# cg-saarland/hagrid

Measured on AMD Instinct MI355X. Metric: Mrays/s (primary traversal) + grid build ms, 1M-tri scene @1/2/4/8 MI355X, higher is better.
Workload: dtype f32

## Files before the change

hagrid_amd/csrc/ctx.h:

```cpp
#pragma once

#include <hip/hip_runtime.h>

#include <atomic>
#include <cstdio>
#include <memory>
#include <string>
#include <unordered_map>
#include <vector>

#include "hagrid_amd.h"

namespace hagrid_impl {

struct Slot {
    void* ptr = nullptr;
    size_t size = 0;
    bool in_use = false;
    int refs = 0;
};

}

namespace hagrid_impl {
// ... 60 lines not shown
enum DistanceScratch : int { kScrDistTasks = 0, kScrDistTooLarge = 1 };
enum ImageScratch : int {
    kScrImgStatus = 160,
    kScrImgLevelCounts = 164,
    kScrImgClearedWords = 24,
    kScrImgTableTotal = 224,
    kScrImgSlimStatus = 228,
};
constexpr bool scr_apart(int a, int na, int b, int nb) { return a + na <= b || b + nb <= a; }
constexpr bool scr_free(int a, int n) { return a >= 0 && a + n <= kScrRowLenBinned; }
static_assert(kScrRowLenBinned + 2 <= kScrRowLen && kScrRowLen + 4 <= kScrMaxRef && kScrMaxRef < kScrBlobFlag && kScrBlobFlag < kScratchWords, "fixed-owner words");
static_assert(kScrBuildTooLarge + 1 <= kScrBuildLevelTotals && kScrBuildShift + 8 == kScrBuildLevelTotals + 1, "build_grid: scalars and the first level's total");
static_assert(scr_apart(kScrBuildLevelTotals, 4 * kBuildMaxLevels, kScrBuildCarry, 2 * kBuildMaxLevels), "build_grid: totals and carries");
static_assert(scr_free(kScrBuildLevelTotals, 4 * kBuildMaxLevels) && scr_free(kScrBuildCarry, 2 * kBuildMaxLevels), "build_grid: level-indexed words");
static_assert(kScrMergeTotals + 6 <= kScrMergeBooks && kScrMergeBooks + 4 == kScrMergeSnapshots && kScrMergeSnapshots + 6 == kScrMergeIpTotal && scr_free(kScrMergeIpTotal, 2), "merge_grid");
static_assert(scr_free(kScrFlattenCarry, HAGRID_MAX_LEVELS + 2), "flatten_grid: a carry per group of levels");
static_assert(scr_free(kScrExpandCounts, kExpandMaxListed), "expand_grid");
static_assert(kScrDistTasks + 1 == kScrDistTooLarge && scr_free(kScrDistTasks, 2) && scr_free(kScrCompressTotal, 1), "distance_lattice (its two words are cleared together), compress_grid");
static_assert(kScrImgStatus + 3 <= kScrImgLevelCounts && kScrImgLevelCounts + kImageMaxLevels + 1 <= kScrImgStatus + kScrImgClearedWords, "setup_traversal: the general layout's words are cleared together");
static_assert(scr_apart(kScrImgStatus, kScrImgClearedWords, kScrImgTableTotal, 1) && scr_apart(kScrImgTableTotal, 1, kScrImgSlimStatus, 3) && scr_free(kScrImgSlimStatus, 3), "setup_traversal");
}

struct hagrid_ctx {
    int device = 0;
    hipStream_t stream = nullptr;
    bool keep = false;
    int num_cus = 0;

    std::vector<hagrid_impl::Slot> slots;
    std::unordered_map<void*, int> tracker;
    size_t usage = 0, max_usage = 0;

    hipEvent_t ev_begin = nullptr, ev_end = nullptr;

    int* mailbox = nullptr;
    int* dscratch = nullptr;
    unsigned long long* lb_state = nullptr;
    size_t lb_words = 0;
    unsigned lb_epoch = 0;
    int* row_scores = nullptr;
    int* bin_diff = nullptr;

    int ray_binning = 0;
    int opt_variant = 0;
    int opt_lookback = 1;
    int opt_merge_inplace = 1;
    int opt_merge_inplace_iters = 0;
    int opt_merge_inplace_div = 0;
    int opt_merge_inplace_room = 0;
    int opt_merge_narrow = 1;
    int opt_expand_voxel_map = 1;
    int opt_expand_subset_only = 1;
    int opt_expand_listed = 1;
    int opt_expand_max_listed = hagrid_impl::kExpandMaxListed;
    int opt_distance_by_triangle = 0;
    int opt_image_width = 0;
    int opt_band_rows = 0;
    int opt_super_log2 = 3;
    int opt_xcd_chunk_log2 = -2;
    int opt_narrow = 1;
    int opt_image_max_mb = 0;
    int opt_quad_head = 20;
    int opt_image_vtop = 1;
    int opt_image_uniform = 1;
    int opt_row_cache = 1;
    struct RayHints {
        const void* key_rays = nullptr; int key_n = 0;
        unsigned long long used = 0;
        struct Rows {
            const void* rowlen_rays = nullptr; int rowlen_n = 0, rowlen_age = 0;
            int rowlen_known = -1, rowlen_seen = 0;
            bool rows_from_origins = false;
            hipEvent_t rowlen_evt = nullptr; bool rowlen_pending = false;
        } rows;
        struct Order {
            int* lpt_buf = nullptr; int lpt_cap = 0;
            const void* lpt_rays = nullptr; int lpt_n = 0, lpt_blocks = 0, lpt_age = 0, lpt_period = 32;
            int lpt_rot = 0;
            bool lpt_valid = false; int lpt_epoch = 1;
            unsigned order_serial = 0; int last_report = -1;
            unsigned long long relearn_clock = 0; int cooldown = 0, cooldown_len = 64;
        } order;
        struct Trial {
            bool rot_adopted = false, head_disabled = false;
            float t_base = 0.0f, t_head = 0.0f, t_all = 0.0f; int n_base = 0, n_head = 0, n_all = 0;
            bool learned_all = false; int all_stage = 0;
            bool cmp_pending = false, cmp_done = false;
            int n_conf = 0; float t_conf = 0.0f;
        } trial;
        hipEvent_t trial_evt[2] = {nullptr, nullptr}; bool trial_pending = false; int trial_kind = 0;
        int trial_opt = -1; unsigned head_serial = 0;
        struct Share {
            hipEvent_t share_evt[12][2] = {}; int share_issued = 0, share_done = 0;
            int share_choice = -1;
            int share_ncand = 0, share_shape_nc = 0;
            int share_cands[4] = {0, 0, 0, 0}; float share_t[4] = {0.0f, 0.0f, 0.0f, 0.0f};
            int share_last = -1;
            int share_launches = 0; unsigned share_serial = 0;
            bool learned_once = false;
            bool order_loses = false;
        } share;
    };
    static constexpr int kRayHints = 4;
    RayHints hints[kRayHints];
    unsigned long long hint_clock = 0;
    int opt_mailbox = -1;
// ... 108 lines not shown
```

hagrid_amd/csrc/expand.hip:

```cpp
#include "ctx.h"
#include "wave_prims.h"

#include "hagrid/grid.h"
#include "hagrid/prims.h"

using namespace hagrid;
using namespace hagrid_impl;

namespace {

struct ExpandK { ivec3 dims; ivec3 top; int shift; vec3 gmin, cell_size, grid_inv; const int* voxel_cells; };
constexpr int kChanged = 1 << 3;
struct CellRec { ivec3 lo; int begin; ivec3 hi; int end; };

__device__ __forceinline__ CellRec load_cell(const Cell* cells, int i) {
    const int4* p = reinterpret_cast<const int4*>(cells) + 2 * size_t(i);
    const int4 a = p[0], b = p[1];
    CellRec c; c.lo = ivec3(a.x, a.y, a.z); c.begin = a.w; c.hi = ivec3(b.x, b.y, b.z); c.end = b.w;
    return c;
}
__device__ __forceinline__ int comp(const ivec3& v, int axis) { return axis == 0 ? v.x : (axis == 1 ? v.y : v.z); }


__device__ __forceinline__ int lower_bound_in(const int* __restrict__ a, int n, int x) {
    int lo = 0, hi = n;
    while (lo < hi) {
        const int mid = (lo + hi) >> 1;
        if (a[mid] < x) lo = mid + 1; else hi = mid;
    }
    return lo;
}

__device__ __forceinline__ bool contains_all(const int* __restrict__ big, int nbig, const int* __restrict__ small, int nsmall) {
    if (nsmall > nbig) return false;
    if (nsmall == 0) return true;
    if (nbig <= 4) {
        const int b0 = big[0], b1 = nbig > 1 ? big[1] : -1, b2 = nbig > 2 ? big[2] : -1, b3 = nbig > 3 ? big[3] : -1;
        const int s0 = small[0], s1 = nsmall > 1 ? small[1] : s0, s2 = nsmall > 2 ? small[2] : s0, s3 = nsmall > 3 ? small[3] : s0;
        auto in_big = [&](int x) { return (x == b0) | (x == b1) | (x == b2) | (x == b3); };
        return in_big(s0) & in_big(s1) & in_big(s2) & in_big(s3);
    }
    for (int j = 0; j < nsmall; j++) {
        const int x = small[j], at = lower_bound_in(big, nbig, x);
        if (at == nbig || big[at] != x) return false;
    }
    return true;
}

__device__ __forceinline__ Tri load_tri(const float4* __restrict__ tris, int i) {
    const float4* p = tris + 3 * size_t(i);
    const float4 a = p[0], b = p[1], c = p[2];
    return Tri(vec3(a.x, a.y, a.z), a.w, vec3(b.x, b.y, b.z), b.w, vec3(c.x, c.y, c.z), c.w);
}

__global__ void __launch_bounds__(kBlock) fill_voxel_cells(ExpandK k, const Entry* __restrict__ entries, int* __restrict__ voxel_cells, int voxels) {
    const int v = blockIdx.x * kBlock + threadIdx.x;
    if (v >= voxels) return;
    const int s = k.shift, m = (1 << s) - 1, top = v >> (3 * s), local = v & ((1 << (3 * s)) - 1);
    const int tx = top % k.top.x, ty = (top / k.top.x) % k.top.y, tz = top / (k.top.x * k.top.y);
    const ivec3 at((tx << s) + (local & m), (ty << s) + ((local >> s) & m), (tz << s) + (local >> (2 * s)));
    voxel_cells[v] = int(lookup_entry(entries, s, k.top, at));
}
__device__ __forceinline__ int cell_of_voxel(const ExpandK& k, const Entry* __restrict__ entries, const ivec3& at) {
    if (!k.voxel_cells) return int(lookup_entry(entries, k.shift, k.top, at));
    const int s = k.shift, m = (1 << s) - 1;
    const int top = (at.x >> s) + k.top.x * ((at.y >> s) + k.top.y * (at.z >> s));
    return k.voxel_cells[(top << (3 * s)) + (at.x & m) + (((at.y & m) + ((at.z & m) << s)) << s)];
}

template <int AXIS>
__device__ __forceinline__ int room_before_prim(const ExpandK& k, const Tri& prim, const CellRec& cell, const BBox& cross, int room, bool UP) {
    constexpr int A1 = (AXIS + 1) % 3, A2 = (AXIS + 2) % 3;
    const BBox pb = prim.bbox();
    const bool overlaps = get<A1>(pb.min) <= get<A1>(cross.max) && get<A1>(pb.max) >= get<A1>(cross.min) &&
                          get<A2>(pb.min) <= get<A2>(cross.max) && get<A2>(pb.max) >= get<A2>(cross.min);
    if (!overlaps) return room;
    const int layer = int(((UP ? get<AXIS>(pb.min) : get<AXIS>(pb.max)) - get<AXIS>(k.gmin)) * get<AXIS>(k.grid_inv));
    const int free_layers = UP ? layer - comp(cell.hi, AXIS) : comp(cell.lo, AXIS) - layer - 1;
    return max(min(room, free_layers), 0);
}

template <int AXIS, bool SUBSET_ONLY>
__device__ __forceinline__ int face_growth(const ExpandK& k, const Entry* __restrict__ entries, const int* __restrict__ refs, const float4* __restrict__ tris,
                                           const Cell* __restrict__ cells, const CellRec& cell, bool UP, bool& again) {
    constexpr int A1 = (AXIS + 1) % 3, A2 = (AXIS + 2) % 3;
    const int face = UP ? comp(cell.hi, AXIS) : comp(cell.lo, AXIS);
    const int extent = comp(k.dims, AXIS);
    if (UP ? face >= extent : face <= 0) return 0;
    const int layer = UP ? face : face - 1;
    const int lo1 = comp(cell.lo, A1), hi1 = comp(cell.hi, A1), lo2 = comp(cell.lo, A2), hi2 = comp(cell.hi, A2);
    const int own = cell.end - cell.begin;
    int reach = extent, room = extent;
    int u = lo1, v = lo2, row_step = comp(k.dims, A2);
    for (;;) {
        const ivec3 at = AXIS == 0 ? ivec3(layer, u, v) : (AXIS == 1 ? ivec3(v, layer, u) : ivec3(u, v, layer));
        const CellRec nb = load_cell(cells, cell_of_voxel(k, entries, at));
        reach = min(reach, UP ? comp(nb.hi, AXIS) - face : face - comp(nb.lo, AXIS));
        room = min(room, reach);
        const int theirs = nb.end - nb.begin;
        if (SUBSET_ONLY) {
            if (!contains_all(refs + cell.begin, own, refs + nb.begin, theirs)) { room = 0; break; }
        } else if (theirs > 0) {
            const BBox cross(k.gmin + k.cell_size * vec3(cell.lo), k.gmin + k.cell_size * vec3(cell.hi));
            int mine = 0;
            for (int j = 0; j < theirs && room > 0; j++) {
                const int id = refs[nb.begin + j];
                while (mine < own && refs[cell.begin + mine] < id) mine++;
                if (mine < own && refs[cell.begin + mine] == id) continue;
                room = room_before_prim<AXIS>(k, load_tri(tris, id), cell, cross, room, UP);
            }
            if (room == 0) break;
        }
        row_step = min(row_step, comp(nb.hi, A2) - v);
        u = comp(nb.hi, A1);
        if (u >= hi1) {
            u = lo1; v += row_step; row_step = comp(k.dims, A2);
            if (v >= hi2) break;
        }
    }
    again |= room == reach;
    return UP ? room : -room;
}

template <int axis, bool SUBSET_ONLY, bool PAIRED>
__device__ __forceinline__ void grow_cell(const ExpandK& k, const Entry* __restrict__ entries, const int* __restrict__ refs, const float4* __restrict__ tris,
                                          const Cell* __restrict__ cells, Cell* __restrict__ new_cells, unsigned char* __restrict__ cell_flags, int id, int flags, bool up) {
    CellRec cell = load_cell(cells, id);
    bool flag = false;
    int ov1, ov2;
    if (PAIRED) {
        bool again = false;
        const int mine = face_growth<axis, SUBSET_ONLY>(k, entries, refs, tris, cells, cell, up, again);
        const int other = __shfl_xor(mine, 1, 64);
        flag = again | (__shfl_xor(int(again), 1, 64) != 0);
        if (up) return;
        ov1 = mine; ov2 = other;
    } else {
        ov1 = face_growth<axis, SUBSET_ONLY>(k, entries, refs, tris, cells, cell, false, flag);
        ov2 = face_growth<axis, SUBSET_ONLY>(k, entries, refs, tris, cells, cell, true, flag);
    }
    if (axis == 0) { cell.lo.x += ov1; cell.hi.x += ov2; }
    if (axis == 1) { cell.lo.y += ov1; cell.hi.y += ov2; }
    if (axis == 2) { cell.lo.z += ov1; cell.hi.z += ov2; }
    cell_flags[id] = (unsigned char)((flag ? 1 << axis : 0) | (flags & ~((1 << axis) | kChanged)) | ((ov1 | ov2) ? kChanged : 0));
    int4* out = reinterpret_cast<int4*>(new_cells) + 2 * size_t(id);
    out[0] = make_int4(cell.lo.x, cell.lo.y, cell.lo.z, cell.begin);
    out[1] = make_int4(cell.hi.x, cell.hi.y, cell.hi.z, cell.end);
}

template <int axis, bool SUBSET_ONLY>
__global__ void __launch_bounds__(kBlock) overlap_step(ExpandK k, const Entry* __restrict__ entries, const int* __restrict__ refs,
                                                       const float4* __restrict__ tris, const Cell* __restrict__ cells, Cell* __restrict__ new_cells,
                                                       unsigned char* __restrict__ cell_flags, int num_cells) {
    const int id = xcd_block(blockIdx.x, gridDim.x) * kBlock + threadIdx.x;
    if (id >= num_cells) return;
    const int flags = cell_flags[id];
    if ((flags & (1 << axis)) == 0) {
        const int4* p = reinterpret_cast<const int4*>(cells) + 2 * size_t(id);
        int4* out = reinterpret_cast<int4*>(new_cells) + 2 * size_t(id);
        const int4 a = p[0], b = p[1];
        out[0] = a; out[1] = b;
        if (flags & kChanged) cell_flags[id] = (unsigned char)(flags & ~kChanged);
        return;
    }
    grow_cell<axis, SUBSET_ONLY, false>(k, entries, refs, tris, cells, new_cells, cell_flags, id, flags, false);
}

constexpr int kSelectItems = 16;
constexpr int kSelectTile = kBlock * kSelectItems;

template <int axis>
__global__ void __launch_bounds__(kBlock) expand_select(const Cell* __restrict__ cells, Cell* __restrict__ new_cells, unsigned char* __restrict__ cell_flags,
                                                        int num_cells, int* __restrict__ list, int* __restrict__ count) {
    __shared__ int tile_list[kSelectTile];
    __shared__ int tile_count, tile_base;
    if (threadIdx.x == 0) tile_count = 0;
    __syncthreads();
    const int base = blockIdx.x * kSelectTile;
    int fl[kSelectItems];
    #pragma unroll
    for (int j = 0; j < kSelectItems; j++) {
        const int id = base + j * kBlock + threadIdx.x;
        fl[j] = id < num_cells ? cell_flags[id] : 0;
    }
    #pragma unroll
    for (int j = 0; j < kSelectItems; j++) {
        const int id = base + j * kBlock + threadIdx.x;
        const int flags = fl[j];
        const bool listed = (flags & (1 << axis)) != 0;
        const unsigned long long m = __ballot(listed);
        int wbase = 0;
        if (lane_id() == 0 && m) wbase = atomicAdd(&tile_count, __popcll(m));
        wbase = __shfl(wbase, 0, 64);
        if (listed) {
            tile_list[wbase + __popcll(m & ((1ull << lane_id()) - 1ull))] = id;
        } else if (flags & kChanged) {
            const int4* p = reinterpret_cast<const int4*>(cells) + 2 * size_t(id);
            int4* out = reinterpret_cast<int4*>(new_cells) + 2 * size_t(id);
            const int4 a = p[0], b = p[1];
            out[0] = a; out[1] = b;
            cell_flags[id] = (unsigned char)(flags & ~kChanged);
        }
    }
    __syncthreads();
    if (threadIdx.x == 0) tile_base = tile_count ? atomicAdd(count, tile_count) : 0;
    __syncthreads();
    for (int i = threadIdx.x; i < tile_count; i += kBlock) list[tile_base + i] = tile_list[i];
}

template <int axis, bool SUBSET_ONLY>
__global__ void __launch_bounds__(kBlock) expand_listed(ExpandK k, const Entry* __restrict__ entries, const int* __restrict__ refs,
                                                        const float4* __restrict__ tris, const Cell* __restrict__ cells, Cell* __restrict__ new_cells,
                                                        unsigned char* __restrict__ cell_flags, const int* __restrict__ list, const int* __restrict__ count) {
    const int n = *count, active = (2 * n + kBlock - 1) / kBlock;
    if (int(blockIdx.x) >= active) return;
    const int t = xcd_block(blockIdx.x, active) * kBlock + threadIdx.x;
    const int i = t >> 1;
    if (i >= n) return;
    const int id = list[i];
    grow_cell<axis, SUBSET_ONLY, true>(k, entries, refs, tris, cells, new_cells, cell_flags, id, cell_flags[id], (t & 1) != 0);
}

template <int axis, bool SUBSET_ONLY>
void listed_step(hipStream_t st, const ExpandK& k, const Entry* entries, const int* refs, const float4* tris, const Cell* cells, Cell* other,
                 unsigned char* flags, int n, int* list, int* count) {
    expand_select<axis><<<grid_blocks(n, kSelectTile), kBlock, 0, st>>>(cells, other, flags, n, list, count);
    expand_listed<axis, SUBSET_ONLY><<<grid_blocks(2ll * n, kBlock), kBlock, 0, st>>>(k, entries, refs, tris, cells, other, flags, list, count);
}

template <bool SUBSET_ONLY>
void listed_iteration(hipStream_t st, const ExpandK& k, const Entry* entries, const int* refs, const float4* tris, Cell*& cells, Cell*& other,
                      unsigned char* flags, int n, int* list, int* counts) {
    listed_step<0, SUBSET_ONLY>(st, k, entries, refs, tris, cells, other, flags, n, list, counts + 0); std::swap(cells, other);
    listed_step<1, SUBSET_ONLY>(st, k, entries, refs, tris, cells, other, flags, n, list, counts + 1); std::swap(cells, other);
    listed_step<2, SUBSET_ONLY>(st, k, entries, refs, tris, cells, other, flags, n, list, counts + 2); std::swap(cells, other);
}
template <bool SUBSET_ONLY>
void all_cells_iteration(hagrid_ctx* ctx, const ExpandK& k, const Entry* entries, const int* refs, const float4* tris, Cell*& cells, Cell*& other,
                         unsigned char* flags, int n) {
    hipStream_t st = ctx->stream;
    const int blocks = grid_blocks(n, kBlock);
    overlap_step<0, SUBSET_ONLY><<<blocks, kBlock, 0, st>>>(k, entries, refs, tris, cells, other, flags, n); HG_DBG(ctx); std::swap(cells, other);
    overlap_step<1, SUBSET_ONLY><<<blocks, kBlock, 0, st>>>(k, entries, refs, tris, cells, other, flags, n); HG_DBG(ctx); std::swap(cells, other);
    overlap_step<2, SUBSET_ONLY><<<blocks, kBlock, 0, st>>>(k, entries, refs, tris, cells, other, flags, n); HG_DBG(ctx); std::swap(cells, other);
}

}

extern "C" int hagrid_expand_grid(hagrid_ctx* ctx, hagrid_grid* grid, const void* tris_v, int iters) {
    if (!ctx || !grid) return HAGRID_EINVAL;
    const bool subset_only = ctx->opt_expand_subset_only != 0;
    if (!subset_only && !tris_v && iters > 0) HG_FAIL(ctx, HAGRID_EINVAL, "expand_grid: the precise mode needs the triangles");
    const float4* tris = static_cast<const float4*>(tris_v);
    if (iters <= 0) return HAGRID_OK;
    if (!grid->cells || !grid->entries || !grid->ref_ids) HG_FAIL(ctx, HAGRID_EINVAL, "expand_grid: incomplete (or compressed) grid");
    trav_image_drop(ctx);
    HG_HIP(ctx, hipSetDevice(ctx->device));
    hipStream_t st = ctx->stream;
    ExpandK k;
    k.top = ivec3(grid->dims[0], grid->dims[1], grid->dims[2]);
    k.dims = k.top << grid->shift;
    k.shift = grid->shift;
    {
        const vec3 lo(grid->bbox_min[0], grid->bbox_min[1], grid->bbox_min[2]), ext = vec3(grid->bbox_max[0], grid->bbox_max[1], grid->bbox_max[2]) - lo;
        k.gmin = lo; k.cell_size = ext / vec3(k.dims); k.grid_inv = vec3(k.dims) / ext;
    }
    const int n = grid->num_cells;
    Cell* cells = static_cast<Cell*>(grid->cells);
    Cell* other = pool_alloc<Cell>(ctx, size_t(n));
    unsigned char* flags = pool_alloc<unsigned char>(ctx, size_t(n));
    if (!other || !flags) { hagrid_mem_free(ctx, other); hagrid_mem_free(ctx, flags); return HAGRID_ENOMEM; }
    (void)hipMemsetAsync(flags, 0xFF, size_t(n), st);
    const Entry* entries = static_cast<const Entry*>(grid->entries);
    const int* refs = static_cast<const int*>(grid->ref_ids);
    int* list = iters > 1 && ctx->opt_expand_listed ? pool_try_alloc<int>(ctx, size_t(n)) : nullptr;
    const long long voxels = (long long)k.dims.x * k.dims.y * k.dims.z;
    int* voxel_cells = (ctx->opt_expand_voxel_map && voxels <= (1ll << 28)) ? pool_try_alloc<int>(ctx, size_t(voxels)) : nullptr;
    k.voxel_cells = voxel_cells;
    if (voxel_cells) { ExpandK kf = k; kf.voxel_cells = nullptr; fill_voxel_cells<<<grid_blocks(voxels, kBlock), kBlock, 0, st>>>(kf, entries, voxel_cells, int(voxels)); HG_DBG(ctx); }
    int* counts = ctx->dscratch + kScrExpandCounts;
    const int max_listed = std::min(std::max(ctx->opt_expand_max_listed, 0), kExpandMaxListed);
    if (list) (void)hipMemsetAsync(counts, 0, kExpandMaxListed * sizeof(int), st);
    int listed = 0;
    for (int it = 0; it < iters; it++) {
        if (it > 0 && list && listed + 3 <= max_listed) {
            if (subset_only) listed_iteration<true>(st, k, entries, refs, tris, cells, other, flags, n, list, counts + listed);
            else             listed_iteration<false>(st, k, entries, refs, tris, cells, other, flags, n, list, counts + listed);
            listed += 3;
            continue;
        }
        if (subset_only) all_cells_iteration<true>(ctx, k, entries, refs, tris, cells, other, flags, n);
        else             all_cells_iteration<false>(ctx, k, entries, refs, tris, cells, other, flags, n);
    }
    hipError_t e = hipGetLastError();
    if (e == hipSuccess) e = hipStreamSynchronize(st);
    ctx->counts.expand_passes = 3 * iters; ctx->counts.expand_cells = n;
    hagrid_mem_free(ctx, flags);
    hagrid_mem_free(ctx, other);
    hagrid_mem_free(ctx, list);
    hagrid_mem_free(ctx, voxel_cells);
    grid->cells = cells;
    if (e != hipSuccess) HG_FAIL(ctx, HAGRID_EHIP, hipGetErrorString(e));
    return HAGRID_OK;
}
```

hagrid_amd/csrc/kat/kat.hip:

```cpp
#include "../trav_kernels.h"
#include "hagrid_amd_kat.h"

#include <cstring>

using namespace hagrid;
using namespace hagrid_impl;
using namespace hagrid_trav;


namespace {

__global__ void kat_prim_ray(const Tri* tris, const Ray* rays, const int* idx, int n, int* ret, int* hid, float* ht) {
    const int i = blockIdx.x * blockDim.x + threadIdx.x;
    if (i >= n) return;
    Hit h(-1, rays[i].tmax, 0, 0);
    ret[i] = intersect_prim_ray(tris[idx[i]], rays[i], idx[i], h) ? 1 : 0;
    hid[i] = h.id; ht[i] = h.t;
}
__global__ void kat_prim_ray_uvs(const Tri* tris, const Ray* rays, const int* idx, int n, int* ret, int* hid, float* ht, float* hu, float* hv) {
    const int i = blockIdx.x * blockDim.x + threadIdx.x;
    if (i >= n) return;
    Hit h(-1, rays[i].tmax, 0, 0);
    ret[i] = intersect_prim_ray_uvs(tris[idx[i]], rays[i], idx[i], h) ? 1 : 0;
    hid[i] = h.id; ht[i] = h.t; hu[i] = h.u; hv[i] = h.v;
// ... 252 lines not shown
    memset(&a, 0, sizeof(a));
    a.num_rays = num_rays; a.row_len_hint = row_len; a.super_log2 = super_log2 & 0xff; a.band_rows = super_log2 >> 8; a.xcd_chunk_log2 = xcd_chunk_log2;
    Staged o(ctx, nullptr, size_t(blocks) * 64 * 4);
    if (!o.d) return HAGRID_ENOMEM;
    kat_tile_slots<<<blocks, 64, 0, ctx->stream>>>(a, (int*)o.d); HG_DBG(ctx);
    HG_HIP(ctx, hipGetLastError());
    return o.fetch(slots);
}

extern "C" int hagrid_kat_image_records(hagrid_ctx* ctx, const hagrid_grid* grid, const int32_t* voxels3, int n, uint32_t* records8, int64_t* image_bytes) {
    if (!ctx || !grid || n < 0) return HAGRID_EINVAL;
    if (!trav_image_matches(ctx, grid)) HG_FAIL(ctx, HAGRID_EINVAL, "no traversal image for this grid");
    if (image_bytes) *image_bytes = (int64_t)ctx->image.block_bytes + (int64_t)ctx->image.table_bytes;
    if (n == 0) return HAGRID_OK;
    TraverseArgs a;
    HG_TRY(make_args(ctx, grid, nullptr, nullptr, nullptr, 0, a));
    image_args(ctx, a);
    Staged v(ctx, voxels3, size_t(n) * 12), o(ctx, nullptr, size_t(n) * 32);
    if (!v.d || !o.d) return HAGRID_ENOMEM;
    kat_image_records<<<grid_blocks(n, 64), 64, 0, ctx->stream>>>(a, (const int*)v.d, n, (uint32_t*)o.d, 1, ctx->image.slim, ctx->image.uniform ? 1 : 0, ctx->image.general ? 1 : 0); HG_DBG(ctx);
    HG_HIP(ctx, hipGetLastError());
    return o.fetch(records8);
}

extern "C" int hagrid_kat_traverse_timed(hagrid_ctx* ctx, const hagrid_grid* grid, const void* tris, const void* rays, void* hits, int num_rays,
                                         int row_len, int tail, unsigned long long* times_dev, const int* tile_order_dev) {
    if (!ctx || !grid || !times_dev || num_rays <= 0) return HAGRID_EINVAL;
    if (!trav_image_matches(ctx, grid) || !(ctx->image.uniform && ctx->image.slim == 20))
        HG_FAIL(ctx, HAGRID_EINVAL, "kat_traverse_timed: needs the table-free image with 20-bit slim records of this grid");
    TraverseArgs a;
    HG_TRY(make_args(ctx, grid, tris, rays, hits, num_rays, a));
    image_args(ctx, a);
    a.row_len_hint = row_len; a.wave_times = times_dev; a.tile_order = tile_order_dev;
    const int blocks = grid_blocks(num_rays, 64);
    if (tail) traverse_kernel_tail<20, true><<<blocks, 64, 0, ctx->stream>>>(a);
    else      traverse_kernel_img<0, 20, 0, true><<<blocks, 64, 0, ctx->stream>>>(a);
    HG_DBG(ctx);
    HG_HIP(ctx, hipGetLastError());
    return HAGRID_OK;
}

extern "C" int hagrid_kat_set_option(hagrid_ctx* ctx, const char* key, int value) {
    if (!ctx || !key) return HAGRID_EINVAL;
    struct { const char* name; int* dst; int lo, hi; } table[] = {
        {"traverse.variant", &ctx->opt_variant, 0, 4},              {"traverse.narrow", &ctx->opt_narrow, 0, 1},
        {"traverse.image_uniform", &ctx->opt_image_uniform, 0, 2},  {"traverse.image_slim", &ctx->opt_image_slim, 1, 2}, {"traverse.image_general", &ctx->opt_image_general, 0, 2}, {"traverse.image_vtop", &ctx->opt_image_vtop, 0, 1}, {"traverse.quad_head", &ctx->opt_quad_head, 0, 1000}, {"ctx.fast_readback", &ctx->opt_fast_readback, 0, 1},
        {"traverse.tail", &ctx->opt_tail, 0, 1},                    {"traverse.quad_tail", &ctx->opt_quad_tail, -1, 100},
        {"traverse.tail_dual", &ctx->opt_tail_dual, -1, 1},        
        {"traverse.super_tile", &ctx->opt_super_log2, 0, 8},        {"traverse.xcd_chunk", &ctx->opt_xcd_chunk_log2, -2, 16},
        {"traverse.row_cache", &ctx->opt_row_cache, 0, 1},          {"traverse.lds_pad", &ctx->opt_lds_pad, 0, 65536},
        {"merge.narrow_cells", &ctx->opt_merge_narrow, 0, 1},       {"scan.lookback", &ctx->opt_lookback, 1, 2},
        {"traverse.order_gate", &ctx->opt_order_gate, 0, 1}, {"traverse.share_trial", &ctx->opt_share_trial, 0, 1}, {"traverse.band_rows", &ctx->opt_band_rows, 0, 1 << 16}, {"traverse.mailbox", &ctx->opt_mailbox, -1, 1},
        {"merge.inplace", &ctx->opt_merge_inplace, 0, 1},           {"merge.inplace_iters", &ctx->opt_merge_inplace_iters, 0, 1 << 20}, {"merge.inplace_room", &ctx->opt_merge_inplace_room, 0, 0x7fffffff}, {"merge.inplace_div", &ctx->opt_merge_inplace_div, 0, 1 << 20},
        {"expand.voxel_map", &ctx->opt_expand_voxel_map, 0, 1},
        {"expand.listed", &ctx->opt_expand_listed, 0, 1},          {"expand.max_listed", &ctx->opt_expand_max_listed, 0, 48},
        {"distance.by_triangle", &ctx->opt_distance_by_triangle, 0, 1},
        {"mem.fail_request", &ctx->opt_fail_request, 0, 0x7fffffff}, {"mem.fail_malloc", &ctx->opt_fail_malloc, 0, 0x7fffffff}, {"mem.fail_scan", &ctx->opt_fail_scan, 0, 0x7fffffff},
    };
    if (!strcmp(key, "scan.epoch")) {
        if (value < 0 || value > (1 << 30) || unsigned(value) < ctx->lb_epoch) HG_FAIL(ctx, HAGRID_EINVAL, "kat_set_option: scan.epoch is 0 .. 2^30 and never goes back");
        ctx->lb_epoch = unsigned(value);
        return HAGRID_OK;
    }
    for (auto& t : table)
        if (!strcmp(key, t.name)) {
            if (value < t.lo || value > t.hi || (t.dst == &ctx->opt_variant && value == 3)) HG_FAIL(ctx, HAGRID_EINVAL, "kat_set_option: value out of range");
            *t.dst = value;
            return HAGRID_OK;
        }
    return hagrid_set_option(ctx, key, value);
}

extern "C" int hagrid_kat_mem_state(hagrid_ctx* ctx, int64_t out[6]) {
    if (!ctx || !out) return HAGRID_EINVAL;
    int64_t in_use = 0, bytes_in_use = 0, bytes_cached = 0;
    for (const auto& s : ctx->slots) {
        if (s.in_use) { in_use++; bytes_in_use += int64_t(s.size); }
        else if (s.ptr) bytes_cached += int64_t(s.size);
    }
    out[0] = ctx->mem_requests; out[1] = ctx->mem_mallocs; out[2] = in_use; out[3] = int64_t(ctx->tracker.size());
    out[4] = bytes_in_use; out[5] = bytes_cached;
    return HAGRID_OK;
}

extern "C" int hagrid_kat_mem_retry(hagrid_ctx* ctx, int64_t out[4]) {
    if (!ctx || !out) return HAGRID_EINVAL;
    out[0] = ctx->mem_retries; out[1] = ctx->mem_retry_bytes; out[2] = ctx->mem_retry_left; out[3] = ctx->mem_retry_slack;
    return HAGRID_OK;
}

extern "C" int hagrid_kat_mem_pending(hagrid_ctx* ctx, int32_t* fail_request, int32_t* fail_malloc, int32_t* fail_scan) {
    if (!ctx) return HAGRID_EINVAL;
    if (fail_request) *fail_request = ctx->opt_fail_request;
    if (fail_malloc) *fail_malloc = ctx->opt_fail_malloc;
    if (fail_scan) *fail_scan = ctx->opt_fail_scan;
    return HAGRID_OK;
}

extern "C" int hagrid_kat_scan_epoch(hagrid_ctx* ctx, int32_t* epoch) {
    if (!ctx || !epoch) return HAGRID_EINVAL;
    *epoch = int32_t(ctx->lb_epoch);
    return HAGRID_OK;
}

extern "C" int hagrid_kat_order_state(hagrid_ctx* ctx, const void* rays, int32_t* out12, float* ms2 ) {
    if (!ctx || !out12) return HAGRID_EINVAL;
    for (int i = 0; i < 12; i++) out12[i] = 0;
// ... 18 lines not shown
```

Baseline: 7702.

## Use packed cell records with inline reference ids during grid expansion

During the expansion passes, cells are stored in a temporary record form: bounds are packed as 16-bit coordinates in the first 16 bytes and up to four reference ids are inlined in the second 16 bytes. Subset checks against neighbour cells then avoid indirect loads from the reference array, and unchanged cells only copy the first half. The select kernel is also rewritten to read flags vectorised and do a wave scan. A conversion kernel restores the normal cell layout at the end, and the record form only applies when every grid dimension is below 65536.

```diff
diff --git a/hagrid_amd/csrc/ctx.h b/hagrid_amd/csrc/ctx.h
--- a/hagrid_amd/csrc/ctx.h
+++ b/hagrid_amd/csrc/ctx.h
@@ -136,6 +136,7 @@
     int opt_expand_voxel_map = 1;
     int opt_expand_subset_only = 1;
     int opt_expand_listed = 1;
+    int opt_expand_records = 1;
     int opt_expand_max_listed = hagrid_impl::kExpandMaxListed;
     int opt_distance_by_triangle = 0;
     int opt_image_width = 0;
diff --git a/hagrid_amd/csrc/expand.hip b/hagrid_amd/csrc/expand.hip
--- a/hagrid_amd/csrc/expand.hip
+++ b/hagrid_amd/csrc/expand.hip
@@ -11,15 +11,68 @@
 
 struct ExpandK { ivec3 dims; ivec3 top; int shift; vec3 gmin, cell_size, grid_inv; const int* voxel_cells; };
 constexpr int kChanged = 1 << 3;
-struct CellRec { ivec3 lo; int begin; ivec3 hi; int end; };
-
-__device__ __forceinline__ CellRec load_cell(const Cell* cells, int i) {
-    const int4* p = reinterpret_cast<const int4*>(cells) + 2 * size_t(i);
+
+__device__ __forceinline__ int comp(const ivec3& v, int axis) { return axis == 0 ? v.x : (axis == 1 ? v.y : v.z); }
+
+struct Node { ivec3 lo, hi; int begin, count; int4 ids; };
+constexpr int kLongList = -2;
+
+__device__ __forceinline__ int id_at(const int4& ids, int j) { return j == 0 ? ids.x : (j == 1 ? ids.y : (j == 2 ? ids.z : ids.w)); }
+
+struct CellForm {
+    static constexpr bool kHalfStores = false;
+    static __device__ __forceinline__ Node load(const Cell* cells, int i) {
+        const int4* p = reinterpret_cast<const int4*>(cells) + 2 * size_t(i);
+        const int4 a = p[0], b = p[1];
+        Node c; c.lo = ivec3(a.x, a.y, a.z); c.begin = a.w; c.hi = ivec3(b.x, b.y, b.z); c.count = b.w - a.w; c.ids = make_int4(-1, -1, -1, -1);
+        return c;
+    }
+    static __device__ __forceinline__ void fetch_ids(Node& c, const int* __restrict__ refs) {
+        if (c.count > 4) return;
+        const int* r = refs + c.begin;
+        c.ids = make_int4(c.count > 0 ? r[0] : -1, c.count > 1 ? r[1] : -1, c.count > 2 ? r[2] : -1, c.count > 3 ? r[3] : -1);
+    }
+    static __device__ __forceinline__ void store(Cell* out, int i, const Node& c, bool) {
+        int4* o = reinterpret_cast<int4*>(out) + 2 * size_t(i);
+        o[0] = make_int4(c.lo.x, c.lo.y, c.lo.z, c.begin);
+        o[1] = make_int4(c.hi.x, c.hi.y, c.hi.z, c.begin + c.count);
+    }
+};
+
+struct RecordForm {
+    static constexpr bool kHalfStores = true;
+    static __device__ __forceinline__ Node load(const Cell* cells, int i) {
+        const int4* p = reinterpret_cast<const int4*>(cells) + 2 * size_t(i);
+        const int4 a = p[0], b = p[1];
+        const unsigned x = unsigned(a.x), y = unsigned(a.y), z = unsigned(a.z);
+        Node c; c.lo = ivec3(int(x & 0xffffu), int(x >> 16), int(y & 0xffffu)); c.hi = ivec3(int(y >> 16), int(z & 0xffffu), int(z >> 16)); c.begin = a.w;
+        const bool is_long = b.x == kLongList;
+        c.count = is_long ? b.y : int(b.x >= 0) + int(b.y >= 0) + int(b.z >= 0) + int(b.w >= 0);
+        c.ids = is_long ? make_int4(-1, -1, -1, -1) : b;
+        return c;
+    }
+    static __device__ __forceinline__ void fetch_ids(Node&, const int* __restrict__) {}
+    static __device__ __forceinline__ void store(Cell* out, int i, const Node& c, bool whole) {
+        int4* o = reinterpret_cast<int4*>(out) + 2 * size_t(i);
+        o[0] = make_int4(int(unsigned(c.lo.x) | (unsigned(c.lo.y) << 16)), int(unsigned(c.lo.z) | (unsigned(c.hi.x) << 16)), int(unsigned(c.hi.y) | (unsigned(c.hi.z) << 16)), c.begin);
+        if (whole) o[1] = c.count > 4 ? make_int4(kLongList, c.count, 0, 0) : c.ids;
+    }
+};
+
+__device__ __forceinline__ void copy_through(const Cell* __restrict__ cells, Cell* __restrict__ new_cells, int id, bool half) {
+    const int4* p = reinterpret_cast<const int4*>(cells) + 2 * size_t(id);
+    int4* out = reinterpret_cast<int4*>(new_cells) + 2 * size_t(id);
+    if (half) { out[0] = p[0]; return; }
     const int4 a = p[0], b = p[1];
-    CellRec c; c.lo = ivec3(a.x, a.y, a.z); c.begin = a.w; c.hi = ivec3(b.x, b.y, b.z); c.end = b.w;
-    return c;
-}
-__device__ __forceinline__ int comp(const ivec3& v, int axis) { return axis == 0 ? v.x : (axis == 1 ? v.y : v.z); }
+    out[0] = a; out[1] = b;
+}
+
+__global__ void __launch_bounds__(kBlock) expand_convert(Cell* cells, int num_cells) {
+    const int i = blockIdx.x * kBlock + threadIdx.x;
+    if (i >= num_cells) return;
+    const Node c = RecordForm::load(cells, i);
+    CellForm::store(cells, i, c, true);
+}
 
 
 __device__ __forceinline__ int lower_bound_in(const int* __restrict__ a, int n, int x) {
@@ -31,18 +84,20 @@
     return lo;
 }
 
-__device__ __forceinline__ bool contains_all(const int* __restrict__ big, int nbig, const int* __restrict__ small, int nsmall) {
-    if (nsmall > nbig) return false;
-    if (nsmall == 0) return true;
-    if (nbig <= 4) {
-        const int b0 = big[0], b1 = nbig > 1 ? big[1] : -1, b2 = nbig > 2 ? big[2] : -1, b3 = nbig > 3 ? big[3] : -1;
-        const int s0 = small[0], s1 = nsmall > 1 ? small[1] : s0, s2 = nsmall > 2 ? small[2] : s0, s3 = nsmall > 3 ? small[3] : s0;
-        auto in_big = [&](int x) { return (x == b0) | (x == b1) | (x == b2) | (x == b3); };
-        return in_big(s0) & in_big(s1) & in_big(s2) & in_big(s3);
-    }
-    for (int j = 0; j < nsmall; j++) {
-        const int x = small[j], at = lower_bound_in(big, nbig, x);
-        if (at == nbig || big[at] != x) return false;
+template <class Form>
+__device__ __forceinline__ bool holds_all_of(const Node& cell, Node& nb, const int* __restrict__ refs) {
+    if (nb.count > cell.count) return false;
+    if (nb.count == 0) return true;
+    Form::fetch_ids(nb, refs);
+    if (cell.count <= 4) {
+        const int4 o = cell.ids;
+        auto in_own = [&](int x) { return (x < 0) | (x == o.x) | (x == o.y) | (x == o.z) | (x == o.w); };
+        return in_own(nb.ids.x) & in_own(nb.ids.y) & in_own(nb.ids.z) & in_own(nb.ids.w);
+    }
+    const int* own = refs + cell.begin;
+    for (int j = 0; j < nb.count; j++) {
+        const int x = nb.count <= 4 ? id_at(nb.ids, j) : refs[nb.begin + j], at = lower_bound_in(own, cell.count, x);
+        if (at == cell.count || own[at] != x) return false;
     }
     return true;
 }
@@ -69,7 +124,7 @@
 }
 
 template <int AXIS>
-__device__ __forceinline__ int room_before_prim(const ExpandK& k, const Tri& prim, const CellRec& cell, const BBox& cross, int room, bool UP) {
+__device__ __forceinline__ int room_before_prim(const ExpandK& k, const Tri& prim, const Node& cell, const BBox& cross, int room, bool UP) {
     constexpr int A1 = (AXIS + 1) % 3, A2 = (AXIS + 2) % 3;
     const BBox pb = prim.bbox();
     const bool overlaps = get<A1>(pb.min) <= get<A1>(cross.max) && get<A1>(pb.max) >= get<A1>(cross.min) &&
@@ -80,33 +135,38 @@
     return max(min(room, free_layers), 0);
 }
 
-template <int AXIS, bool SUBSET_ONLY>
+template <class Form, int AXIS, bool SUBSET_ONLY>
 __device__ __forceinline__ int face_growth(const ExpandK& k, const Entry* __restrict__ entries, const int* __restrict__ refs, const float4* __restrict__ tris,
-                                           const Cell* __restrict__ cells, const CellRec& cell, bool UP, bool& again) {
+                                           const Cell* __restrict__ cells, const Node& cell, bool UP, bool& again) {
     constexpr int A1 = (AXIS + 1) % 3, A2 = (AXIS + 2) % 3;
     const int face = UP ? comp(cell.hi, AXIS) : comp(cell.lo, AXIS);
     const int extent = comp(k.dims, AXIS);
     if (UP ? face >= extent : face <= 0) return 0;
     const int layer = UP ? face : face - 1;
     const int lo1 = comp(cell.lo, A1), hi1 = comp(cell.hi, A1), lo2 = comp(cell.lo, A2), hi2 = comp(cell.hi, A2);
-    const int own = cell.end - cell.begin;
+    const int own = cell.count;
     int reach = extent, room = extent;
     int u = lo1, v = lo2, row_step = comp(k.dims, A2);
     for (;;) {
         const ivec3 at = AXIS == 0 ? ivec3(layer, u, v) : (AXIS == 1 ? ivec3(v, layer, u) : ivec3(u, v, layer));
-        const CellRec nb = load_cell(cells, cell_of_voxel(k, entries, at));
+        Node nb = Form::load(cells, cell_of_voxel(k, entries, at));
         reach = min(reach, UP ? comp(nb.hi, AXIS) - face : face - comp(nb.lo, AXIS));
         room = min(room, reach);
-        const int theirs = nb.end - nb.begin;
+        const int theirs = nb.count;
         if (SUBSET_ONLY) {
-            if (!contains_all(refs + cell.begin, own, refs + nb.begin, theirs)) { room = 0; break; }
+            if (!holds_all_of<Form>(cell, nb, refs)) { room = 0; break; }
         } else if (theirs > 0) {
             const BBox cross(k.gmin + k.cell_size * vec3(cell.lo), k.gmin + k.cell_size * vec3(cell.hi));
+            Form::fetch_ids(nb, refs);
             int mine = 0;
             for (int j = 0; j < theirs && room > 0; j++) {
-                const int id = refs[nb.begin + j];
-                while (mine < own && refs[cell.begin + mine] < id) mine++;
-                if (mine < own && refs[cell.begin + mine] == id) continue;
+                const int id = theirs <= 4 ? id_at(nb.ids, j) : refs[nb.begin + j];
+                int at_mine = -1;
+                for (; mine < own; mine++) {
+                    at_mine = own <= 4 ? id_at(cell.ids, mine) : refs[cell.begin + mine];
+                    if (at_mine >= id) break;
+                }
+                if (mine < own && at_mine == id) continue;
                 room = room_before_prim<AXIS>(k, load_tri(tris, id), cell, cross, room, UP);
             }
             if (room == 0) break;
@@ -122,127 +182,188 @@
     return UP ? room : -room;
 }
 
-template <int axis, bool SUBSET_ONLY, bool PAIRED>
+template <class Form, class Out, int axis, bool SUBSET_ONLY, bool PAIRED>
 __device__ __forceinline__ void grow_cell(const ExpandK& k, const Entry* __restrict__ entries, const int* __restrict__ refs, const float4* __restrict__ tris,
-                                          const Cell* __restrict__ cells, Cell* __restrict__ new_cells, unsigned char* __restrict__ cell_flags, int id, int flags, bool up) {
-    CellRec cell = load_cell(cells, id);
+                                          const Cell* __restrict__ cells, Cell* __restrict__ new_cells, unsigned char* __restrict__ cell_flags, int id, int flags, bool up, bool whole) {
+    Node cell = Form::load(cells, id);
+    Form::fetch_ids(cell, refs);
     bool flag = false;
     int ov1, ov2;
     if (PAIRED) {
         bool again = false;
-        const int mine = face_growth<axis, SUBSET_ONLY>(k, entries, refs, tris, cells, cell, up, again);
+        const int mine = face_growth<Form, axis, SUBSET_ONLY>(k, entries, refs, tris, cells, cell, up, again);
         const int other = __shfl_xor(mine, 1, 64);
         flag = again | (__shfl_xor(int(again), 1, 64) != 0);
         if (up) return;
         ov1 = mine; ov2 = other;
     } else {
-        ov1 = face_growth<axis, SUBSET_ONLY>(k, entries, refs, tris, cells, cell, false, flag);
-        ov2 = face_growth<axis, SUBSET_ONLY>(k, entries, refs, tris, cells, cell, true, flag);
+        ov1 = face_growth<Form, axis, SUBSET_ONLY>(k, entries, refs, tris, cells, cell, false, flag);
+        ov2 = face_growth<Form, axis, SUBSET_ONLY>(k, entries, refs, tris, cells, cell, true, flag);
     }
     if (axis == 0) { cell.lo.x += ov1; cell.hi.x += ov2; }
     if (axis == 1) { cell.lo.y += ov1; cell.hi.y += ov2; }
     if (axis == 2) { cell.lo.z += ov1; cell.hi.z += ov2; }
     cell_flags[id] = (unsigned char)((flag ? 1 << axis : 0) | (flags & ~((1 << axis) | kChanged)) | ((ov1 | ov2) ? kChanged : 0));
-    int4* out = reinterpret_cast<int4*>(new_cells) + 2 * size_t(id);
-    out[0] = make_int4(cell.lo.x, cell.lo.y, cell.lo.z, cell.begin);
-    out[1] = make_int4(cell.hi.x, cell.hi.y, cell.hi.z, cell.end);
-}
-
-template <int axis, bool SUBSET_ONLY>
-__global__ void __launch_bounds__(kBlock) overlap_step(ExpandK k, const Entry* __restrict__ entries, const int* __restrict__ refs,
-                                                       const float4* __restrict__ tris, const Cell* __restrict__ cells, Cell* __restrict__ new_cells,
-                                                       unsigned char* __restrict__ cell_flags, int num_cells) {
+    Out::store(new_cells, id, cell, whole);
+}
+
+template <class Form, class Out, int axis, bool SUBSET_ONLY>
+__device__ __forceinline__ void all_cells_pass(const ExpandK& k, const Entry* __restrict__ entries, const int* __restrict__ refs, const float4* __restrict__ tris,
+                                               const Cell* __restrict__ cells, Cell* __restrict__ new_cells, unsigned char* __restrict__ cell_flags, int num_cells, bool whole) {
+    constexpr bool same_form = Form::kHalfStores == Out::kHalfStores;
+    whole = whole || !Out::kHalfStores;
     const int id = xcd_block(blockIdx.x, gridDim.x) * kBlock + threadIdx.x;
     if (id >= num_cells) return;
     const int flags = cell_flags[id];
     if ((flags & (1 << axis)) == 0) {
-        const int4* p = reinterpret_cast<const int4*>(cells) + 2 * size_t(id);
-        int4* out = reinterpret_cast<int4*>(new_cells) + 2 * size_t(id);
-        const int4 a = p[0], b = p[1];
-        out[0] = a; out[1] = b;
+        if (same_form) {
+            copy_through(cells, new_cells, id, !whole);
+        } else {
+            Node cell = Form::load(cells, id);
+            Form::fetch_ids(cell, refs);
+            Out::store(new_cells, id, cell, true);
+        }
         if (flags & kChanged) cell_flags[id] = (unsigned char)(flags & ~kChanged);
         return;
     }
-    grow_cell<axis, SUBSET_ONLY, false>(k, entries, refs, tris, cells, new_cells, cell_flags, id, flags, false);
+    grow_cell<Form, Out, axis, SUBSET_ONLY, false>(k, entries, refs, tris, cells, new_cells, cell_flags, id, flags, false, whole || !same_form);
+}
+
+template <int axis, bool SUBSET_ONLY>
+__global__ void __launch_bounds__(kBlock) overlap_step(ExpandK k, const Entry* __restrict__ entries, const int* __restrict__ refs,
+                                                       const float4* __restrict__ tris, const Cell* __restrict__ cells, Cell* __restrict__ new_cells,
+                                                       unsigned char* __restrict__ cell_flags, int num_cells, int from_cells, int whole) {
+    if (axis == 0 && from_cells) all_cells_pass<CellForm, RecordForm, axis, SUBSET_ONLY>(k, entries, refs, tris, cells, new_cells, cell_flags, num_cells, true);
+    else                         all_cells_pass<RecordForm, RecordForm, axis, SUBSET_ONLY>(k, entries, refs, tris, cells, new_cells, cell_flags, num_cells, whole != 0);
 }
 
 constexpr int kSelectItems = 16;
 constexpr int kSelectTile = kBlock * kSelectItems;
 
-template <int axis>
 __global__ void __launch_bounds__(kBlock) expand_select(const Cell* __restrict__ cells, Cell* __restrict__ new_cells, unsigned char* __restrict__ cell_flags,
-                                                        int num_cells, int* __restrict__ list, int* __restrict__ count) {
-    __shared__ int tile_list[kSelectTile];
-    __shared__ int tile_count, tile_base;
-    if (threadIdx.x == 0) tile_count = 0;
+                                                        int num_cells, int* __restrict__ list, int* __restrict__ count, int axis, int half) {
+    __shared__ int wave_total[kWaves];
+    __shared__ int tile_base;
+    __shared__ uint4 tile_flags[kBlock];
+    const int first = (blockIdx.x * kBlock + threadIdx.x) * kSelectItems;
+    const bool whole = first + kSelectItems <= num_cells;
+    unsigned w[4] = {0u, 0u, 0u, 0u};
+    if (whole) {
+        const uint4 v = *reinterpret_cast<const uint4*>(cell_flags + first);
+        w[0] = v.x; w[1] = v.y; w[2] = v.z; w[3] = v.w;
+    } else {
+        for (int j = 0; first + j < num_cells; j++) w[j >> 2] |= unsigned(cell_flags[first + j]) << (8 * (j & 3));
+    }
+    unsigned listed[4], stale[4];
+    int mine = 0;
+    unsigned any_stale = 0u;
+    #pragma unroll
+    for (int q = 0; q < 4; q++) {
+        listed[q] = (w[q] >> axis) & 0x01010101u;
+        stale[q] = (w[q] >> 3) & ~listed[q] & 0x01010101u;
+        mine += __popc(listed[q]);
+        any_stale |= stale[q];
+    }
+    tile_flags[threadIdx.x] = make_uint4(w[0], w[1], w[2], w[3]);
+    const int incl = wave_inclusive_scan(mine);
+    if (lane_id() == 63) wave_total[wave_id()] = incl;
     __syncthreads();
-    const int base = blockIdx.x * kSelectTile;
-    int fl[kSelectItems];
+    int before = 0, total = 0;
+    #pragma unroll
+    for (int v = 0; v < kWaves; v++) { const int t = wave_total[v]; before += v < wave_id() ? t : 0; total += t; }
+    if (threadIdx.x == 0) tile_base = total ? atomicAdd(count, total) : 0;
+    const unsigned char* flag_of = reinterpret_cast<const unsigned char*>(tile_flags);
     #pragma unroll
     for (int j = 0; j < kSelectItems; j++) {
-        const int id = base + j * kBlock + threadIdx.x;
-        fl[j] = id < num_cells ? cell_flags[id] : 0;
-    }
+        const int c = j * kBlock + threadIdx.x, f = flag_of[c];
+        if (((f >> axis) & 1) == 0 && (f & kChanged) != 0) copy_through(cells, new_cells, blockIdx.x * kSelectTile + c, half != 0);
+    }
+    if (any_stale) {
+        if (whole) {
+            *reinterpret_cast<uint4*>(cell_flags + first) = make_uint4(w[0] & ~(stale[0] << 3), w[1] & ~(stale[1] << 3), w[2] & ~(stale[2] << 3), w[3] & ~(stale[3] << 3));
+        } else {
+            for (int j = 0; first + j < num_cells; j++)
+                if ((stale[j >> 2] >> (8 * (j & 3))) & 1u) cell_flags[first + j] = (unsigned char)((w[j >> 2] >> (8 * (j & 3))) & 0xffu & ~unsigned(kChanged));
+        }
+    }
+    __syncthreads();
+    if (mine == 0) return;
+    int at = tile_base + before + incl - mine;
     #pragma unroll
-    for (int j = 0; j < kSelectItems; j++) {
-        const int id = base + j * kBlock + threadIdx.x;
-        const int flags = fl[j];
-        const bool listed = (flags & (1 << axis)) != 0;
-        const unsigned long long m = __ballot(listed);
-        int wbase = 0;
-        if (lane_id() == 0 && m) wbase = atomicAdd(&tile_count, __popcll(m));
-        wbase = __shfl(wbase, 0, 64);
-        if (listed) {
-            tile_list[wbase + __popcll(m & ((1ull << lane_id()) - 1ull))] = id;
-        } else if (flags & kChanged) {
-            const int4* p = reinterpret_cast<const int4*>(cells) + 2 * size_t(id);
-            int4* out = reinterpret_cast<int4*>(new_cells) + 2 * size_t(id);
-            const int4 a = p[0], b = p[1];
-            out[0] = a; out[1] = b;
-            cell_flags[id] = (unsigned char)(flags & ~kChanged);
-        }
-    }
-    __syncthreads();
-    if (threadIdx.x == 0) tile_base = tile_count ? atomicAdd(count, tile_count) : 0;
-    __syncthreads();
-    for (int i = threadIdx.x; i < tile_count; i += kBlock) list[tile_base + i] = tile_list[i];
-}
-
-template <int axis, bool SUBSET_ONLY>
-__global__ void __launch_bounds__(kBlock) expand_listed(ExpandK k, const Entry* __restrict__ entries, const int* __restrict__ refs,
-                                                        const float4* __restrict__ tris, const Cell* __restrict__ cells, Cell* __restrict__ new_cells,
-                                                        unsigned char* __restrict__ cell_flags, const int* __restrict__ list, const int* __restrict__ count) {
+    for (int j = 0; j < kSelectItems; j++)
+        if ((listed[j >> 2] >> (8 * (j & 3))) & 1u) list[at++] = first + j;
+}
+
+template <class Form, int axis, bool SUBSET_ONLY>
+__device__ __forceinline__ void listed_pass(const ExpandK& k, const Entry* __restrict__ entries, const int* __restrict__ refs, const float4* __restrict__ tris,
+                                            const Cell* __restrict__ cells, Cell* __restrict__ new_cells, unsigned char* __restrict__ cell_flags,
+                                            const int* __restrict__ list, const int* __restrict__ count) {
     const int n = *count, active = (2 * n + kBlock - 1) / kBlock;
     if (int(blockIdx.x) >= active) return;
     const int t = xcd_block(blockIdx.x, active) * kBlock + threadIdx.x;
     const int i = t >> 1;
     if (i >= n) return;
     const int id = list[i];
-    grow_cell<axis, SUBSET_ONLY, true>(k, entries, refs, tris, cells, new_cells, cell_flags, id, cell_flags[id], (t & 1) != 0);
+    grow_cell<Form, Form, axis, SUBSET_ONLY, true>(k, entries, refs, tris, cells, new_cells, cell_flags, id, cell_flags[id], (t & 1) != 0, !Form::kHalfStores);
 }
 
 template <int axis, bool SUBSET_ONLY>
-void listed_step(hipStream_t st, const ExpandK& k, const Entry* entries, const int* refs, const float4* tris, const Cell* cells, Cell* other,
-                 unsigned char* flags, int n, int* list, int* count) {
-    expand_select<axis><<<grid_blocks(n, kSelectTile), kBlock, 0, st>>>(cells, other, flags, n, list, count);
-    expand_listed<axis, SUBSET_ONLY><<<grid_blocks(2ll * n, kBlock), kBlock, 0, st>>>(k, entries, refs, tris, cells, other, flags, list, count);
+__global__ void __launch_bounds__(kBlock) expand_listed(ExpandK k, const Entry* __restrict__ entries, const int* __restrict__ refs,
+                                                        const float4* __restrict__ tris, const Cell* __restrict__ cells, Cell* __restrict__ new_cells,
+                                                        unsigned char* __restrict__ cell_flags, const int* __restrict__ list, const int* __restrict__ count) {
+    listed_pass<RecordForm, axis, SUBSET_ONLY>(k, entries, refs, tris, cells, new_cells, cell_flags, list, count);
+}
+
+template <int axis, bool SUBSET_ONLY>
+__device__ __forceinline__ void cell_form_pass(const ExpandK& k, const Entry* __restrict__ entries, const int* __restrict__ refs, const float4* __restrict__ tris,
+                                               const Cell* __restrict__ cells, Cell* __restrict__ new_cells, unsigned char* __restrict__ cell_flags, int num_cells,
+                                               const int* __restrict__ list, const int* __restrict__ count) {
+    if (list) listed_pass<CellForm, axis, SUBSET_ONLY>(k, entries, refs, tris, cells, new_cells, cell_flags, list, count);
+    else      all_cells_pass<CellForm, CellForm, axis, SUBSET_ONLY>(k, entries, refs, tris, cells, new_cells, cell_flags, num_cells, true);
+}
+__global__ void __launch_bounds__(kBlock) expand_cell_form(ExpandK k, const Entry* __restrict__ entries, const int* __restrict__ refs,
+                                                           const float4* __restrict__ tris, const Cell* __restrict__ cells, Cell* __restrict__ new_cells,
+                                                           unsigned char* __restrict__ cell_flags, int num_cells, const int* __restrict__ list, const int* __restrict__ count,
+                                                           int axis, int subset_only) {
+    switch (2 * axis + (subset_only ? 1 : 0)) {
+        case 0: cell_form_pass<0, false>(k, entries, refs, tris, cells, new_cells, cell_flags, num_cells, list, count); break;
+        case 1: cell_form_pass<0, true>(k, entries, refs, tris, cells, new_cells, cell_flags, num_cells, list, count); break;
+        case 2: cell_form_pass<1, false>(k, entries, refs, tris, cells, new_cells, cell_flags, num_cells, list, count); break;
+        case 3: cell_form_pass<1, true>(k, entries, refs, tris, cells, new_cells, cell_flags, num_cells, list, count); break;
+        case 4: cell_form_pass<2, false>(k, entries, refs, tris, cells, new_cells, cell_flags, num_cells, list, count); break;
+        default: cell_form_pass<2, true>(k, entries, refs, tris, cells, new_cells, cell_flags, num_cells, list, count); break;
+    }
+}
+
+struct Passes {
+    hagrid_ctx* ctx; ExpandK k; const Entry* entries; const int* refs; const float4* tris; Cell* cells; Cell* other; unsigned char* flags; int n;
+    bool records;
+    int done;
+};
+
+template <int axis, bool SUBSET_ONLY>
+void run_pass(Passes& p, int* list, int* count) {
+    hipStream_t st = p.ctx->stream;
+    if (list) {
+        const int blocks = grid_blocks(2ll * p.n, kBlock);
+        expand_select<<<grid_blocks(p.n, kSelectTile), kBlock, 0, st>>>(p.cells, p.other, p.flags, p.n, list, count, axis, p.records ? 1 : 0);
+        if (p.records) expand_listed<axis, SUBSET_ONLY><<<blocks, kBlock, 0, st>>>(p.k, p.entries, p.refs, p.tris, p.cells, p.other, p.flags, list, count);
+        else           expand_cell_form<<<blocks, kBlock, 0, st>>>(p.k, p.entries, p.refs, p.tris, p.cells, p.other, p.flags, p.n, list, count, axis, SUBSET_ONLY ? 1 : 0);
+    } else {
+        const int blocks = grid_blocks(p.n, kBlock);
+        if (p.records) overlap_step<axis, SUBSET_ONLY><<<blocks, kBlock, 0, st>>>(p.k, p.entries, p.refs, p.tris, p.cells, p.other, p.flags, p.n, p.done == 0, p.done < 2);
+        else           expand_cell_form<<<blocks, kBlock, 0, st>>>(p.k, p.entries, p.refs, p.tris, p.cells, p.other, p.flags, p.n, nullptr, nullptr, axis, SUBSET_ONLY ? 1 : 0);
+        HG_DBG(p.ctx);
+    }
+    std::swap(p.cells, p.other);
+    p.done++;
 }
 
 template <bool SUBSET_ONLY>
-void listed_iteration(hipStream_t st, const ExpandK& k, const Entry* entries, const int* refs, const float4* tris, Cell*& cells, Cell*& other,
-                      unsigned char* flags, int n, int* list, int* counts) {
-    listed_step<0, SUBSET_ONLY>(st, k, entries, refs, tris, cells, other, flags, n, list, counts + 0); std::swap(cells, other);
-    listed_step<1, SUBSET_ONLY>(st, k, entries, refs, tris, cells, other, flags, n, list, counts + 1); std::swap(cells, other);
-    listed_step<2, SUBSET_ONLY>(st, k, entries, refs, tris, cells, other, flags, n, list, counts + 2); std::swap(cells, other);
-}
-template <bool SUBSET_ONLY>
-void all_cells_iteration(hagrid_ctx* ctx, const ExpandK& k, const Entry* entries, const int* refs, const float4* tris, Cell*& cells, Cell*& other,
-                         unsigned char* flags, int n) {
-    hipStream_t st = ctx->stream;
-    const int blocks = grid_blocks(n, kBlock);
-    overlap_step<0, SUBSET_ONLY><<<blocks, kBlock, 0, st>>>(k, entries, refs, tris, cells, other, flags, n); HG_DBG(ctx); std::swap(cells, other);
-    overlap_step<1, SUBSET_ONLY><<<blocks, kBlock, 0, st>>>(k, entries, refs, tris, cells, other, flags, n); HG_DBG(ctx); std::swap(cells, other);
-    overlap_step<2, SUBSET_ONLY><<<blocks, kBlock, 0, st>>>(k, entries, refs, tris, cells, other, flags, n); HG_DBG(ctx); std::swap(cells, other);
+void run_iteration(Passes& p, int* list, int* counts) {
+    run_pass<0, SUBSET_ONLY>(p, list, counts + 0);
+    run_pass<1, SUBSET_ONLY>(p, list, counts + 1);
+    run_pass<2, SUBSET_ONLY>(p, list, counts + 2);
 }
 
 }
@@ -281,17 +402,17 @@
     int* counts = ctx->dscratch + kScrExpandCounts;
     const int max_listed = std::min(std::max(ctx->opt_expand_max_listed, 0), kExpandMaxListed);
     if (list) (void)hipMemsetAsync(counts, 0, kExpandMaxListed * sizeof(int), st);
+    const bool records = ctx->opt_expand_records && voxel_cells && std::max(k.dims.x, std::max(k.dims.y, k.dims.z)) < 65536;
+    Passes p{ctx, k, entries, refs, tris, cells, other, flags, n, records, 0};
     int listed = 0;
     for (int it = 0; it < iters; it++) {
-        if (it > 0 && list && listed + 3 <= max_listed) {
-            if (subset_only) listed_iteration<true>(st, k, entries, refs, tris, cells, other, flags, n, list, counts + listed);
-            else             listed_iteration<false>(st, k, entries, refs, tris, cells, other, flags, n, list, counts + listed);
-            listed += 3;
-            continue;
-        }
-        if (subset_only) all_cells_iteration<true>(ctx, k, entries, refs, tris, cells, other, flags, n);
-        else             all_cells_iteration<false>(ctx, k, entries, refs, tris, cells, other, flags, n);
-    }
+        const bool from_list = it > 0 && list && listed + 3 <= max_listed;
+        if (subset_only) run_iteration<true>(p, from_list ? list : nullptr, counts + listed);
+        else             run_iteration<false>(p, from_list ? list : nullptr, counts + listed);
+        if (from_list) listed += 3;
+    }
+    cells = p.cells; other = p.other;
+    if (records) { expand_convert<<<grid_blocks(n, kBlock), kBlock, 0, st>>>(cells, n); HG_DBG(ctx); }
     hipError_t e = hipGetLastError();
     if (e == hipSuccess) e = hipStreamSynchronize(st);
     ctx->counts.expand_passes = 3 * iters; ctx->counts.expand_cells = n;
diff --git a/hagrid_amd/csrc/kat/kat.hip b/hagrid_amd/csrc/kat/kat.hip
--- a/hagrid_amd/csrc/kat/kat.hip
+++ b/hagrid_amd/csrc/kat/kat.hip
@@ -328,7 +328,7 @@
         {"merge.narrow_cells", &ctx->opt_merge_narrow, 0, 1},       {"scan.lookback", &ctx->opt_lookback, 1, 2},
         {"traverse.order_gate", &ctx->opt_order_gate, 0, 1}, {"traverse.share_trial", &ctx->opt_share_trial, 0, 1}, {"traverse.band_rows", &ctx->opt_band_rows, 0, 1 << 16}, {"traverse.mailbox", &ctx->opt_mailbox, -1, 1},
         {"merge.inplace", &ctx->opt_merge_inplace, 0, 1},           {"merge.inplace_iters", &ctx->opt_merge_inplace_iters, 0, 1 << 20}, {"merge.inplace_room", &ctx->opt_merge_inplace_room, 0, 0x7fffffff}, {"merge.inplace_div", &ctx->opt_merge_inplace_div, 0, 1 << 20},
-        {"expand.voxel_map", &ctx->opt_expand_voxel_map, 0, 1},
+        {"expand.voxel_map", &ctx->opt_expand_voxel_map, 0, 1},     {"expand.records", &ctx->opt_expand_records, 0, 1},
         {"expand.listed", &ctx->opt_expand_listed, 0, 1},          {"expand.max_listed", &ctx->opt_expand_max_listed, 0, 48},
         {"distance.by_triangle", &ctx->opt_distance_by_triangle, 0, 1},
         {"mem.fail_request", &ctx->opt_fail_request, 0, 0x7fffffff}, {"mem.fail_malloc", &ctx->opt_fail_malloc, 0, 0x7fffffff}, {"mem.fail_scan", &ctx->opt_fail_scan, 0, 0x7fffffff},
```

After: 7695. No clear change (-0.1%).
